# markokr/libacm

Hardware: AMD Instinct MI355X
Metric: decoded PCM Msamples/sec over a batch of ACM streams (hot path on HBM-resident staged input) (higher is better)
Workload: dtype int32

## Files before the change

### libacm_amd/csrc/acm_device.h

```cpp
#ifndef ACM_DEVICE_H
#define ACM_DEVICE_H

#include <stdint.h>

#include "acm_hip.h"

struct AcmDevStream {
	uint64_t idx_off;
	uint64_t hdr_off;
	uint64_t pcm_off;
	uint64_t n_emit;
	uint64_t scratch_off;
	uint32_t level;
	uint32_t rows;
	uint32_t nrows;
	uint32_t row_begin;
	uint32_t halo_row;
	uint32_t pad;
};

struct AcmTile {
	uint32_t stream;
	int32_t row0;
	uint32_t flags;
	uint32_t pad;
};
#define ACM_TILE_FRESH   1u
#define ACM_TILE_DISCARD 2u
#define ACM_TILE_ROW1    4u
#define ACM_TILE_ODD     8u
#define ACM_TILE_ONEBLOCK 16u

struct AcmTile2 {
	uint64_t idx_off;
	uint64_t pcm_off;
	uint32_t hdr_blk;
	uint32_t rowpos;
	uint32_t magic;
	uint32_t flags;
};

struct AcmDevPatch {
	uint64_t dst;
	int32_t value;
	uint32_t pad;
};

struct AcmParseJob {
	uint64_t file_off;
	uint64_t idx_off;
	uint64_t hdr_off;
	uint64_t col_off;
	uint32_t file_len;
	uint32_t data_start;
	uint32_t level;
	uint32_t rows;
	uint32_t blocks;
	uint32_t range_unit;
	uint64_t mf_off;
	uint32_t mf_pair_off;
	uint32_t mf_rows;
};
struct AcmParseResult {
	uint32_t blocks_done;
	uint32_t status;
	uint32_t end_bit;
	uint32_t mf_at;
};

struct AcmBlockJob {
	uint32_t job;
	uint32_t block;
	uint32_t bit;
	uint32_t end_bit;
	uint32_t h20;
	uint32_t pad;
};

#define ACM_K1_MIN_LEVEL 5
#define ACM_K1_MAX_LEVEL 12
#define ACM_K2_MIN_LEVEL 6
#define ACM_K2_MAX_LEVEL 14
#define ACM_K2P_MIN_LEVEL 6
#define ACM_K2P_MAX_LEVEL 9
// ... 112 lines not shown
```

### libacm_amd/csrc/acm_hip_api.cpp

```cpp
#include <hip/hip_runtime.h>

#include <cstdarg>
#include <cstdio>
#include <cstdlib>
#include <cstring>
#include <mutex>
#include <new>
#include <vector>

#include "acm_device.h"
#include "acm_hip.h"
#include "acm_plan_cut.h"

namespace {

thread_local char g_err[512] = "";

void set_err(const char *fmt, ...)
{
	va_list ap;
	va_start(ap, fmt);
	vsnprintf(g_err, sizeof(g_err), fmt, ap);
	va_end(ap);
}
// ... 472 lines not shown
	}
	if (plan->ev_fork)
		(void)hipEventDestroy(plan->ev_fork);
	for (hipEvent_t e : plan->ev_join)
		if (e)
			(void)hipEventDestroy(e);
	if (plan->dev) {
		acmhip_device *dev = plan->dev;
		std::vector<acmhip_device::Block> drop;
		{
			std::lock_guard<std::mutex> g(dev->spare_mutex);
			for (const acmhip_device::Block &b : plan->blocks) {
				if (dev->spare.size() < acmhip_device::SPARE_MAX_BLOCKS && dev->spare_bytes + b.bytes <= acmhip_device::SPARE_MAX_BYTES &&
				    b.bytes <= acmhip_device::SPARE_MAX_BYTES / 4) {
					dev->spare.push_back(b);
					dev->spare_bytes += b.bytes;
				} else {
					drop.push_back(b);
				}
			}
		}
		for (const acmhip_device::Block &b : drop)
			(void)hipFree(b.ptr);
	}
	delete plan;
}

extern "C" int acmhip_plan_create(acmhip_device *dev, const acmhip_stream_desc *streams, size_t n,
				  const acmhip_patch *patches, size_t npatches, unsigned flags,
				  acmhip_plan **out)
{
	return acmhip_plan_create_packed(dev, streams, n, nullptr, patches, npatches, flags, out);
}

extern "C" int acmhip_plan_create_packed(acmhip_device *dev, const acmhip_stream_desc *streams, size_t n, const acmhip_packed_stream *packed,
					 const acmhip_patch *patches, size_t npatches, unsigned flags, acmhip_plan **out)
{
	if (!dev || !out || (n && !streams) || (npatches && !patches) || n > 0xFFFFFFFFull)
		return ACMHIP_ERR_ARG;
	HIPTRY(hipSetDevice(dev->ordinal));
	AcmPlanCut cut;
	int rc = acm_plan_cut(dev->cus, streams, n, packed, patches, npatches, flags, &cut);
	if (rc != ACMHIP_OK)
		return rc;

	acmhip_plan *pl = new (std::nothrow) acmhip_plan;
	if (!pl)
		return ACMHIP_ERR_NOMEM;
	pl->dev = dev;
	pl->variant = cut.variant;
	pl->form_only = cut.form_only;
	pl->form_rows = std::move(cut.form_rows);
	pl->stats = cut.stats;
	rc = to_device(pl, cut.streams, &pl->d_streams);
	if (rc == ACMHIP_OK)
		rc = upload_groups(pl, cut.fused, &pl->fused);
	if (rc == ACMHIP_OK)
		rc = upload_groups(pl, cut.small, &pl->small);
	if (rc == ACMHIP_OK)
		rc = upload_groups(pl, cut.prefix, &pl->prefix);
	if (rc == ACMHIP_OK)
		rc = upload_groups(pl, cut.stagewise, &pl->stagewise);
	if (rc == ACMHIP_OK && cut.need_sink)
		rc = plan_malloc(pl, (void **)&pl->d_sink, ACM_K2_SINK_F32_BYTES);
	if (rc == ACMHIP_OK && cut.plane_elems > 0) {
		pl->n_sw_all = (uint32_t)cut.sw_all.size();
		pl->sw_max_elems = cut.sw_max_elems;
		pl->plane_elems = cut.plane_elems;
		pl->npatches = cut.patches.size();
		rc = to_device(pl, cut.sw_all, &pl->d_sw_all);
		if (rc == ACMHIP_OK)
			rc = to_device(pl, cut.patches, &pl->d_patches);
		for (int b = 0; b < 2 && rc == ACMHIP_OK; b++)
			rc = plan_malloc(pl, (void **)&pl->d_plane[b], cut.plane_elems * sizeof(int32_t));
	}
	if (rc == ACMHIP_OK)
		rc = upload_done(pl, (flags & ACMHIP_PLAN_UPLOAD_ASYNC) != 0);
	if (rc != ACMHIP_OK) {
		acmhip_plan_destroy(pl);
		return rc;
	}
	if (pl->fused.size() > 1 && !(ACM_TUNING_ENV("ACM_PLAN_STREAMS") && atoi(ACM_TUNING_ENV("ACM_PLAN_STREAMS")) <= 1)) {
		hipError_t e = hipEventCreateWithFlags(&pl->ev_fork, hipEventDisableTiming);
		for (int k = 0; k < 2 && e == hipSuccess; k++) {
			e = hipEventCreateWithFlags(&pl->ev_join[k], hipEventDisableTiming);
			if (e == hipSuccess && !dev->side[k])
				e = hipStreamCreateWithFlags(&dev->side[k], hipStreamNonBlocking);
		}
		if (e != hipSuccess) {
			rc = hip_fail(e, "side streams of a multi-level plan");
			acmhip_plan_destroy(pl);
			return rc;
		}
	}
	*out = pl;
	return ACMHIP_OK;
}

extern "C" int acmhip_plan_form_rows(const acmhip_plan *plan, size_t stream, uint64_t *rows)
{
	if (!plan || !rows || stream >= plan->form_rows.size())
		return ACMHIP_ERR_ARG;
	*rows = plan->form_rows[stream];
	return ACMHIP_OK;
}

// ... 161 lines not shown
```

### libacm_amd/csrc/acm_kernels.hip

```cpp
#include <hip/hip_runtime.h>

#include <utility>

#include "acm_device.h"

#ifndef ACM_L14_GROUPS
#define ACM_L14_GROUPS 3, 3, 3, 3, 2
#endif
#ifndef ACM_L13_GROUPS
#define ACM_L13_GROUPS 2, 3, 3, 3, 2
#endif

#ifndef ACM_OUT_F32
#define ACM_OUT_F32 0
#endif
#if ACM_OUT_F32
#define ACM_K_EMIT acm_sw_emit_f32
#define ACM_K_SMALL acm_small_level_f32
#define ACM_K_FUSED acm_fused_tile_f32
#define ACM_K_TILE2 acm_f32_tile2
#define ACM_K_CHUNK acm_f32_chunk
#define ACMK_OUT(name) name##_f32
#else
#define ACM_K_EMIT acm_sw_emit
// ... 1986 lines not shown
			e = (u >> 1) >= (uint32_t)j ? (uint32_t)opaque_s((int32_t)d.e[j]) : e;
		return e;
	}

	static constexpr bool HISTORY_IN_REGISTERS = RR == 1;
#ifndef ACM_K3_DPP_HISTORY
#define ACM_K3_DPP_HISTORY 1
#endif
	static constexpr bool HISTORY_BY_DPP = ACM_K3_DPP_HISTORY && RR >= 2 && NSW == 2 && RR * SIGMA == 16 && SIGMA >= 4;
	static constexpr bool KEEPS_ROWS = HISTORY_IN_REGISTERS || HISTORY_BY_DPP;
	template <int CTRL, int BANKS>
	static __device__ __forceinline__ v4u_t dpp4(const v4u_t old, const v4u_t src)
	{
		v4u_t r;
#pragma unroll
		for (int v = 0; v < 4; v++)
			r[v] = (uint32_t)__builtin_amdgcn_update_dpp((int)old[v], (int)src[v], CTRL, 0xF, BANKS, false);
		return r;
	}
	static constexpr int DPP_W0_BANKS = (1 << (SIGMA / 4)) - 1;
	static __device__ __forceinline__ void hand_history_on(Raw &raw)
	{
#pragma unroll
		for (int k = 0; k < 2; k++) {
			raw.lo[0][k] = dpp4<0x100 + (16 - SIGMA), DPP_W0_BANKS>(raw.lo[0][k], raw.lo[0][k + NSW]);
			raw.hi[0][k] = dpp4<0x100 + (16 - SIGMA), DPP_W0_BANKS>(raw.hi[0][k], raw.hi[0][k + NSW]);
		}
	}
	static __device__ __forceinline__ void take_history_from_partner(Raw &raw)
	{
#pragma unroll
		for (int k = 0; k < 2; k++) {
			raw.lo[0][k] = dpp4<0x110 + SIGMA, 0xF & ~DPP_W0_BANKS>(raw.lo[0][k], raw.lo[0][k + NSW]);
			raw.hi[0][k] = dpp4<0x110 + SIGMA, 0xF & ~DPP_W0_BANKS>(raw.hi[0][k], raw.hi[0][k + NSW]);
		}
	}
	static constexpr int JM = (TR & 1) ? 1 : TR / 2;
	static_assert(JM + 1 <= NE, "entries in reach are entries fetched");
	static __device__ __forceinline__ uint32_t half_bytes(const uint32_t cls) { return (0x4234u >> (4u * cls)) & 15u; }
	template <int J0>
	static __device__ __forceinline__ uint32_t mode_of(const uint32_t flags, const Desc &d, const uint32_t sval)
	{
		const uint32_t cls = d.e[0] & 3u;
		const uint32_t pair_units = (uint32_t)(COLS / 64) * half_bytes(cls);
		bool ok = (flags & ACM_TILE_ONEBLOCK) != 0 && cls != 0u;
		if constexpr (OutScale<L>::SHIFT != 0)
			ok = ok && sval < 65536u;
#pragma unroll
		for (int j = 1; j <= JM; j++)
			ok = ok && (d.e[j] & 3u) == cls;
#pragma unroll
		for (int j = J0; j < JM; j++)
			ok = ok && (d.e[j + 1] >> 2) - (d.e[j] >> 2) == pair_units;
		return ok ? (cls == ACMHIP_BP_NIB12 ? 3u : cls - (ACMHIP_BP_BYTE - 1u)) : 0u;
	}

#ifndef ACM_K3_LD_MOD
#define ACM_K3_LD_MOD " nt"
#endif
	template <bool KEEP>
	static __device__ __forceinline__ void issue(Raw &raw, const uint8_t *arena, const Desc &d, const int lane, const uint32_t odd, const uint32_t mode)
	{
		static_assert(!KEEP || KEEPS_ROWS, "the rows in front belong to another lane");
		constexpr int K0 = KEEP ? 2 : 0, J0 = KEEP ? 1 : 0;
		const uint32_t i = (uint32_t)lane & 15u, ks = (uint32_t)lane >> 4;
		const uint32_t c = class_of(i), rr = RR == 1 ? 0u : i / SIGMA;
		const uint32_t smode = __builtin_amdgcn_readfirstlane(mode);
		uint32_t va[NX][NG], vh[NX][NG];
		const uint8_t *sb[NX][NG];
		if (mode) {
			const uint32_t hb = smode == 1u ? 2u : smode == 2u ? 4u : 3u;
			const uint64_t base = reinterpret_cast<uint64_t>(arena) + ((uint64_t)(d.e[J0] >> 2) << 6);
			const uint32_t vl = (rr * (uint32_t)(NSW * COLS / 2) + c * (uint32_t)(QN / 2)) * hb + 16u * ks;
			const uint32_t vlh = vl - (smode == 3u ? 8u * ks : 0u);
#pragma unroll
			for (int k = K0; k < NX; k++)
#pragma unroll
				for (int g = 0; g < NG; g++) {
					va[k][g] = vl;
					vh[k][g] = vlh;
					sb[k][g] = sgpr_u64(base + (uint64_t)((((TR & 1 ? odd : 0u) + (uint32_t)(k - K0)) * (uint32_t)(COLS / 2) + group_at(g) * (uint32_t)(QN / 2)) * hb));
				}
		} else {
			const uint32_t e0 = d.e[0];
			const uint8_t *base = sgpr_u64(reinterpret_cast<uint64_t>(arena) + ((uint64_t)(e0 >> 2) << 6));
#pragma unroll
			for (int k = K0; k < NX; k++) {
				const uint32_t u = (TR & 1 ? odd : 0u) + rr * NSW + k;
				const uint32_t e = entry_of(d, u);
				const uint32_t hb = half_bytes(e & 3u);
				const uint32_t row_at = (((e >> 2) - (e0 >> 2)) << 6) + ((u & 1u) ? (uint32_t)(COLS / 2) * hb : 0u) + 16u * ks;
#pragma unroll
				for (int g = 0; g < NG; g++) {
					va[k][g] = row_at + (group_at(g) + c) * (uint32_t)(QN / 2) * hb;
					vh[k][g] = va[k][g] - ((e & 3u) == ACMHIP_BP_NIB12 ? 8u * ks : 0u);
					sb[k][g] = base;
				}
			}
		}
#pragma unroll
		for (int k = K0; k < NX; k++)
#pragma unroll
			for (int g = 0; g < NG; g++) {
				if constexpr (KEEPS_ROWS) {
					asm volatile("global_load_dwordx4 %0, %1, %2" ACM_K3_LD_MOD : "=v"(raw.lo[g][k]) : "v"(va[k][g]), "s"(sb[k][g]) : "memory");
					asm volatile("s_cmp_eq_u32 %3, 1\n\ts_cbranch_scc1 .Lacm_z8_%=\n\t"
						     "global_load_dwordx4 %0, %1, %2 offset:64" ACM_K3_LD_MOD "\n"
						     ".Lacm_z8_%=:"
						     : "+v"(raw.hi[g][k]) : "v"(vh[k][g]), "s"(sb[k][g]), "s"(smode) : "memory", "scc");
				} else {
					asm volatile("global_load_dwordx4 %0, %1, %2" : "=v"(raw.lo[g][k]) : "v"(va[k][g]), "s"(sb[k][g]) : "memory");
					asm volatile("s_cmp_eq_u32 %3, 1\n\ts_cbranch_scc1 .Lacm_z8_%=\n\t"
						     "global_load_dwordx4 %0, %1, %2 offset:64\n"
						     ".Lacm_z8_%=:"
						     : "+v"(raw.hi[g][k]) : "v"(vh[k][g]), "s"(sb[k][g]), "s"(smode) : "memory", "scc");
				}
			}
	}
	static __device__ __forceinline__ v4u_t expand_nib(const v4u_t x)
	{
// ... 223 lines not shown
#pragma unroll
							for (int v = 0; v < 4; v++)
								y[v] = (int32_t)(__umul24((uint32_t)ha[v], v8[v / NVH]) + (uint32_t)y[v]);
							goto joined;
						}
					}
					{
					v4i_t yh;
					int32_t wv[NH], w2[NH], w1[NH];
#pragma unroll
					for (int hf = 0; hf < NH; hf++) {
						wv[hf] = opaque_v(val[s][hf]);
						w2[hf] = opaque_v(dv2[s][hf]);
						w1[hf] = opaque_v(dv1[s][hf]);
					}
#pragma unroll
					for (int v = 0; v < 4; v++)
						yh[v] = __mul24(ha[v], wv[v / NVH]);
					if (step2[s]) {
#pragma unroll
						for (int v = 0; v < 4; v++)
							yh[v] += __mul24(h2[v], w2[v / NVH]);
					}
					if (step1[s]) {
#pragma unroll
						for (int v = 0; v < 4; v++)
							yh[v] += __mul24(h1[v], w1[v / NVH]);
					}
					const uint32_t hs = nform ? 4u : 8u;
#pragma unroll
					for (int v = 0; v < 4; v++)
						y[v] = (int32_t)(((uint32_t)opaque_v(yh[v]) << hs) + (uint32_t)y[v]);
					}
				joined:;
				}
				}
				static_assert(COLS % (1 << PS) == 0 && (SIGMA * 16) % (1 << PS) == 0 &&
					      (NG == 1 || (group_at(NG - 1) % (1 << PS) + CB + 7 < (1 << PS) && SIGMA % (1 << PS) == 0)), "address split");
#pragma unroll
				for (int hf = 0; hf < NH; hf++) {
					uint32_t *const o = tile + (o_lane[hf] + (uint32_t)((s * COLS + ((s * COLS) >> PS)) + (group_at(g) + (group_at(g) >> PS))));
#pragma unroll
					for (int v = 0; v < NVH; v++)
						o[v] = (uint32_t)y[hf * NVH + v];
				}
			}
			cf += 64;
#pragma unroll
			for (int hf = 0; hf < NH; hf++)
				o_lane[hf] += SIGMA * 16 + ((SIGMA * 16) >> PS);
		}
	}

	static __device__ __forceinline__ void run(Raw &raw, uint32_t *const tile, const Tables &t, const int lane_, const uint32_t hvs,
						   const Desc &d, const uint32_t in_front, const uint32_t odd, const uint32_t mode, const uint32_t sval,
						   const bool first)
	{
#ifdef ACM_K3_OPAQUE_LANE
		const int lane = opaque_v(lane_);
#else
		const int lane = lane_;
#endif
		const bool all_new = !KEEPS_ROWS || first;
		if (mode == 3u) {
#pragma unroll
			for (int k = 0; k < NX; k++)
				if (k >= 2 || all_new) {
#pragma unroll
					for (int g = 0; g < NG; g++)
						raw.hi[g][k] = expand_nib(raw.hi[g][k]);
				}
			if constexpr (HISTORY_BY_DPP)
				take_history_from_partner(raw);
			run_t<true, true, true>(raw, tile, t, lane, 0u, in_front, sval);
			return;
		}
		if (mode) {
			if constexpr (HISTORY_BY_DPP)
				take_history_from_partner(raw);
			if (mode == 2u)
				run_t<true, true>(raw, tile, t, lane, 0u, in_front, sval);
			else
				run_t<false, true>(raw, tile, t, lane, 0u, in_front, sval);
			return;
		}
		uint32_t any_word = 0, any_nib = 0, any_wordu = 0;
#pragma unroll
		for (int j = 0; j < NE; j++) {
			any_word |= (d.e[j] & 3u) == ACMHIP_BP_WORD ? 1u : 0u;
			any_nib |= (d.e[j] & 3u) == ACMHIP_BP_NIB12 ? 1u : 0u;
			any_wordu |= (d.e[j] & 3u) == ACMHIP_BP_WORDU ? 1u : 0u;
		}
		any_word |= any_wordu;
		const uint32_t rr = RR == 1 ? 0u : ((uint32_t)lane & 15u) / SIGMA;
		if (any_nib) {
#pragma unroll
			for (int k = 0; k < NX; k++)
				if (k >= 2 || all_new) {
					if ((entry_of(d, (TR & 1 ? odd : 0u) + rr * NSW + k) & 3u) == ACMHIP_BP_NIB12) {
#pragma unroll
						for (int g = 0; g < NG; g++)
							raw.hi[g][k] = expand_nib(raw.hi[g][k]);
					}
				}
		}
		if constexpr (HISTORY_BY_DPP)
			take_history_from_partner(raw);
		const bool nform = any_nib && !any_word;
		if (any_word | any_nib) {
#pragma unroll
			for (int k = 0; k < NX; k++) {
				const uint32_t cls = entry_of(d, (TR & 1 ? odd : 0u) + rr * NSW + k) & 3u;
				const uint32_t mask = cls == ACMHIP_BP_BYTE ? 0u : 0xFFFFFFFFu;
#pragma unroll
				for (int g = 0; g < NG; g++)
					raw.hi[g][k] &= mask;
// ... 34 lines not shown
	constexpr int PASS_ABL = ABL | MODE_WAVE | (FP::NG > 1 && NW == 16 ? MODE_LEAN : 0);

	__shared__ uint32_t tile_mem[NW][WTILE];
	__shared__ uint32_t carry_all[NW][NCARRY_WORDS];
	__shared__ typename FP::Tables tables;

	const int lane0 = threadIdx.x & 63;
	const uint32_t wave = __builtin_amdgcn_readfirstlane(threadIdx.x >> 6);
	FP::fill_tables(tables, threadIdx.x, NW * 64);
	__syncthreads();

	uint32_t *const tile = tile_mem[wave] + 8;
	uint32_t *const carry_mem = carry_all[wave];

	const uint32_t nvw = gridDim.x * NW, vw = blockIdx.x * NW + wave;
	const uint32_t per = (ntiles + nvw - 1) / nvw;
	uint32_t t = vw * per;
	const uint32_t t_end = t + per < ntiles ? t + per : ntiles;
	if (t >= t_end)
		return;
	bool discard = false;
	{
		const uint32_t f0 = tiles[__builtin_amdgcn_readfirstlane(t)].flags;
		if (f0 & ACM_TILE_DISCARD) {
			discard = true;
		} else if (!(f0 & ACM_TILE_FRESH)) {
			discard = true;
			t--;
		}
	}

	auto rows_in_front = [](const AcmTile2 &r) -> uint32_t { return (r.flags & ACM_TILE_FRESH) ? 0u : (r.flags & ACM_TILE_ROW1) ? 1u : 2u; };
	auto fetch_val = [&](const AcmTile2 &r, const int lane, uint32_t v, const uint32_t mode) -> uint32_t {
		const uint32_t *p = &hdr[0].val;
		if (!mode) {
			const uint32_t lr_fetch = (uint32_t)(lane < TR + 2 ? lane : TR + 1);
			const uint32_t missing = 2u - rows_in_front(r);
			const uint32_t q = r.rowpos + (lr_fetch < missing ? 0u : lr_fetch - missing);
			const uint32_t b = r.magic ? __umulhi(q, r.magic) : q;
			p = &hdr[r.hdr_blk + b].val;
		}
		asm volatile("s_cmp_lg_u32 %2, 0\n\ts_cbranch_scc1 .Lacm_zv_%=\n\t"
			     "global_load_dword %0, %1, off\n"
			     ".Lacm_zv_%=:"
			     : "+v"(v) : "v"(p), "s"(__builtin_amdgcn_readfirstlane(mode)) : "memory", "scc");
		return v;
	};
	typedef const uint32_t __attribute__((address_space(4))) *const_u32_ptr;
	auto val_of = [&](const AcmTile2 &r) -> uint32_t {
		const uint64_t a = reinterpret_cast<uint64_t>(&hdr[__builtin_amdgcn_readfirstlane(r.hdr_blk)].val);
		return *(const_u32_ptr)a << OutScale<L>::SHIFT;
	};

	constexpr int NVEC = TR * COLS / 8, PER_OWNER = NJ_LAST / 8, NSTORE = NVEC / 64;
	static_assert(NVEC % 64 == 0, "whole rounds");
	const uint8_t *const arena = reinterpret_cast<const uint8_t *>(idx);
	auto record_at = [&](const uint32_t k) -> AcmTile2 { return tiles[__builtin_amdgcn_readfirstlane(k < t_end ? k : t_end - 1)]; };
	constexpr int MODE_J0 = FP::KEEPS_ROWS ? 1 : 0;
#ifdef ACM_K3_NO_FAST
	auto mode_of = [&](const AcmTile2 &, const typename FP::Desc &, const uint32_t) -> uint32_t { return 0u; };
#else
	auto mode_of = [&](const AcmTile2 &r, const typename FP::Desc &d, const uint32_t sval) -> uint32_t {
		return FP::template mode_of<MODE_J0>(r.flags, d, sval);
	};
#endif
	AcmTile2 cur = record_at(t);
	typename FP::Desc dcur = FP::fetch_desc(pairs, cur);
	typename FP::Raw raw;
	{
		const v4u_t z = { 0, 0, 0, 0 };
#pragma unroll
		for (int g = 0; g < FP::NG; g++)
#pragma unroll
			for (int k = 0; k < FP::NX; k++)
				raw.hi[g][k] = z;
	}
	uint32_t mode_cur = 0u, sv_cur = val_of(cur);
	uint32_t hv = fetch_val(cur, lane0, 0u, 0u);
	FP::template issue<false>(raw, arena, dcur, lane0, (cur.flags & ACM_TILE_ODD) ? 1u : 0u, 0u);
	k2_wait<0>();
	bool fresh = true, first_of_run = true;
	AcmTile2 nxt = record_at(t + 1), nx2 = record_at(t + 2);
	typename FP::Desc dnxt = FP::fetch_desc(pairs, nxt);
	uint32_t sv_nxt = val_of(nxt);
	uint32_t mode_nxt = mode_of(nxt, dnxt, sv_nxt);
#ifdef ACM_STAMPS
	unsigned long long acc_[8] = { 0, 0, 0, 0, 0, 0, 0, 0 };
	unsigned long long last_ = stamp_now();
#endif
	for (;;) {
		const uint32_t tn = t + 1;
		const bool more = tn < t_end;
		int lane = lane0;
#ifdef ACM_K3_OPAQUE_LANE
		asm volatile("" : "+v"(lane));
#endif
		if (fresh)
			for (int k = lane; k < NCARRY_WORDS; k += 64)
				carry_mem[k] = 0u;
		const uint32_t hvs = hv << OutScale<L>::SHIFT;
		ACM_STAMP(0);
		phase_prio<true, PRIO_FIRST_PASS>();
		FP::run(raw, tile, tables, lane, hvs, dcur, rows_in_front(cur), (cur.flags & ACM_TILE_ODD) ? 1u : 0u, mode_cur, sv_cur, first_of_run);
		first_of_run = false;
		phase_prio<true, PRIO_IDLE>();
		ACM_STAMP(1);

		hv = fetch_val(nxt, lane, hv, mode_nxt);
		if constexpr (FP::HISTORY_IN_REGISTERS) {
			FP::shift_history(raw);
			if (nxt.flags & ACM_TILE_FRESH)
				FP::zero_history(raw);
			FP::template issue<true>(raw, arena, dnxt, lane, (nxt.flags & ACM_TILE_ODD) ? 1u : 0u, mode_nxt);
		} else if constexpr (FP::HISTORY_BY_DPP) {
			FP::hand_history_on(raw);
			if (nxt.flags & ACM_TILE_FRESH)
				FP::zero_history(raw);
			FP::template issue<true>(raw, arena, dnxt, lane, (nxt.flags & ACM_TILE_ODD) ? 1u : 0u, mode_nxt);
		} else {
			FP::template issue<false>(raw, arena, dnxt, lane, (nxt.flags & ACM_TILE_ODD) ? 1u : 0u, mode_nxt);
		}
		const AcmTile2 nx3 = record_at(t + 3);
		const typename FP::Desc dnx2 = FP::fetch_desc(pairs, nx2);
		const uint32_t sv_nx2 = val_of(nx2);
		ACM_STAMP(2);
		phase_prio<true, PRIO_LDS_PASSES>();
		run_lds_passes<C, PASS_ABL, true, FP::G, Gs...>(tile, lane, F32 ? (unsigned)ACMHIP_FMT_S16LE : fmt, carry_mem);
		tile_barrier<MODE_WAVE>();
		ACM_STAMP(3);
		if constexpr (F32) {
			float *out = discard ? reinterpret_cast<float *>(sink) : reinterpret_cast<float *>(pcm) + cur.pcm_off;
			lean_store_f32<C, 64, NSTORE, ABL>(tile, lane, out);
		} else {
			typedef uint32_t v4u __attribute__((ext_vector_type(4)));
			v4u *out = discard ? reinterpret_cast<v4u *>(sink) : reinterpret_cast<v4u *>(reinterpret_cast<uint16_t *>(pcm) + cur.pcm_off);
#pragma unroll
			for (int k = 0; k < NSTORE; k++) {
				const int vec = lane + k * 64;
				const uint32_t *q = tile + lds_at<C::PS>((vec / PER_OWNER) * NJ_LAST) + (vec % PER_OWNER) * park_piece<NJ_LAST>();
				const v4u o = { q[0], q[1], q[2], q[3] };
#ifdef ACM_K3_ST_MOD
				asm volatile("global_store_dwordx4 %0, %1, %2" ACM_K3_ST_MOD :: "v"((uint32_t)(vec * 16)), "v"(o), "s"(sgpr_u64(reinterpret_cast<uint64_t>(out))) : "memory");
#else
				__builtin_nontemporal_store(o, &out[vec]);
#endif
			}
		}
		ACM_STAMP(5);
		phase_prio<true, PRIO_IDLE>();
		k2_wait<F32 ? 2 * NSTORE : NSTORE>();
		ACM_STAMP(6);
		tile_barrier<MODE_WAVE>();
		if (!more)
			break;
		fresh = (nxt.flags & (ACM_TILE_FRESH | ACM_TILE_DISCARD)) != 0;
		discard = (nxt.flags & ACM_TILE_DISCARD) != 0;
		cur = nxt;
		dcur = dnxt;
		sv_cur = sv_nxt;
		mode_cur = mode_nxt;
		t = tn;
		nxt = nx2;
		dnxt = dnx2;
		sv_nxt = sv_nx2;
		mode_nxt = mode_of(nxt, dnxt, sv_nxt);
		nx2 = nx3;
	}
#ifdef ACM_STAMPS
	if (lane0 == 0 && vw < 2048)
		for (int k = 0; k < 8; k++)
			g_acm_stamps[vw][k] = acc_[k];
#endif
}

struct Tile2Entry {
	typedef void (*Fn)(const AcmTile2 *, uint32_t, const int16_t *, const uint32_t *, const acmhip_blkhdr *, int16_t *, int16_t *, unsigned);
	Fn fn;
	int threads, tile_rows, wg_per_cu;
};
template <class C, int... Gs>
constexpr Tile2Entry entry_k2()
{
	return Tile2Entry{ ACM_K_TILE2<C, 4, 0, false, Gs...>, C::NT, C::TR, 1024 / C::NT };
}
template <class C, int WPC, int... Gs>
constexpr Tile2Entry entry_k2w()
{
	return Tile2Entry{ ACM_K_TILE2<C, WPC * C::NT / 256, 0, false, Gs...>, C::NT, C::TR, WPC };
}
#ifdef ACM_ABLATION
template <int ABL>
constexpr Tile2Entry abl_k2() { return Tile2Entry{ ACM_K_TILE2<TileCfg<9, 256, 8192>, 4, ABL, false, 3, 3, 3>, 256, 16, 4 }; }
const struct { int mask; Tile2Entry e; } g_tile2_abl[] = {
	{ 1, abl_k2<1>() }, { 2, abl_k2<2>() }, { 4, abl_k2<4>() }, { 6, abl_k2<6>() }, { 8, abl_k2<8>() }, { 16, abl_k2<16>() },
	{ 17, abl_k2<17>() }, { 23, abl_k2<23>() }, { 32, abl_k2<32>() }, { 25, abl_k2<25>() }, { 31, abl_k2<31>() }, { 12, abl_k2<12>() },
};
#endif
const Tile2Entry g_tile2[ACM_K2_MAX_LEVEL - ACM_K2_MIN_LEVEL + 1] = {
	entry_k2<TileCfg<6, 256, 8192>, 2, 2, 2>(),
	entry_k2<TileCfg<7, 256, 8192>, 3, 2, 2>(),
	entry_k2<TileCfg<8, 256, 8192>, 3, 3, 2>(),
	entry_k2<TileCfg<9, 256, 8192>, 3, 3, 3>(),
	entry_k2<TileCfg<10, 256, 8192>, 3, 3, 2, 2>(),
	entry_k2<TileCfg<11, 256, 8192>, 3, 3, 3, 2>(),
	entry_k2w<TileCfg<12, 512, 16384>, 2, 3, 3, 3, 3>(),
	entry_k2w<TileCfg<13, 1024, 32768>, 1, ACM_L13_GROUPS>(),
	entry_k2w<TileCfg<14, 1024, 32768>, 1, ACM_L14_GROUPS>(),
};
inline const Tile2Entry &tile2_entry(uint32_t level)
{
	return g_tile2[level - ACM_K2_MIN_LEVEL];
}
template <class C, int... Gs>
constexpr Tile2Entry entry_k2m()
{
	return Tile2Entry{ ACM_K_TILE2<C, 4, 0, true, Gs...>, C::NT, C::TR, 1024 / C::NT };
}
// ... 731 lines not shown
```

### libacm_amd/csrc/acm_plan_cut.cpp

```cpp
#include <algorithm>
#include <cstdarg>
#include <cstdio>
#include <cstdlib>
#include <cstring>

#include "acm_plan_cut.h"

#define ACM_K1_DEFAULT_VARIANT 0

namespace {

void set_err(const char *fmt, ...)
{
	char text[512];
	va_list ap;
	va_start(ap, fmt);
	vsnprintf(text, sizeof(text), fmt, ap);
	va_end(ap);
	acmhip_set_error_text(text);
}

bool fused_ok(const acmhip_stream_desc &s, int variant)
{
	return s.level >= ACM_K1_MIN_LEVEL && s.level <= ACM_K1_MAX_LEVEL && acmk_fused_tile_rows(s.level, variant) > 2;
// ... 513 lines not shown
			g.carry = carry_wanted(L.prefix_tiles_carry.size(), (size_t)acmk_plane_grid(cus), (size_t)acmk_plane_tile_rows(), flags);
			g.tiles = std::move(g.carry ? L.prefix_tiles_carry : L.prefix_tiles);
			st.tiles += g.tiles.size();
			st.launches += g.prefix_patched ? 2 + g.prefix_stages : 2;
			cut.prefix.push_back(std::move(g));
		}
		if (!L.list.empty()) {
			AcmCutGroup g;
			g.level = level;
			g.max_elems = L.max_elems;
			g.max_emit = L.max_emit;
			g.list = std::move(L.list);
			cut.stagewise.push_back(std::move(g));
			st.launches += level + 1;
		}
	}
	if (cut.plane_elems > 0) {
		st.launches += cut.sw_all.empty() ? 0 : 1;
		st.launches += cut.patches.empty() ? 0 : 1;
	}
}

int Cutter::run()
{
	int rc = index_patches();
	if (rc != ACMHIP_OK)
		return rc;
	cut.streams.resize(n);
	cut.form_rows.assign(n, 0);
	cut.variant = variant;
	cut.form_only = (flags & ACMHIP_PLAN_FORM_ONLY) != 0;
	plane_shift.assign(n, 0);
	on_tile_kernel.assign(n, 0);
	count_high_levels();
	for (size_t i = 0; i < n && rc == ACMHIP_OK; i++)
		rc = cut_stream(i);
	if (rc == ACMHIP_OK)
		rc = resolve_patches();
	if (rc == ACMHIP_OK)
		choose_tables();
	return rc;
}

}

int acm_plan_cut(int cus, const acmhip_stream_desc *streams, size_t n, const acmhip_packed_stream *packed,
		 const acmhip_patch *patches, size_t npatches, unsigned flags, AcmPlanCut *out)
{
	if (!out || (n && !streams) || (npatches && !patches) || n > 0xFFFFFFFFull)
		return ACMHIP_ERR_ARG;
	*out = AcmPlanCut{};
	Cutter c(cus, streams, n, packed, patches, npatches, flags, *out);
	return c.run();
}

extern "C" int acmk_plan_cut_visit(int cus, const acmhip_stream_desc *streams, size_t n, const acmhip_packed_stream *packed,
				   const acmhip_patch *patches, size_t npatches, unsigned flags, acmk_cut_visit visit, void *ctx)
{
	AcmPlanCut cut;
	const int rc = acm_plan_cut(cus, streams, n, packed, patches, npatches, flags, &cut);
	if (rc != ACMHIP_OK || !visit)
		return rc;
	auto show = [&](const char *name, uint32_t level, const auto &v) {
		if (!v.empty())
			visit(ctx, name, level, v.data(), sizeof(v[0]), v.size());
	};
	show("streams", 0, cut.streams);
	const std::vector<AcmCutGroup> *kinds[4] = { &cut.fused, &cut.small, &cut.prefix, &cut.stagewise };
	static const char *const list_name[4] = { "", "small_list", "prefix_list", "sw_list" };
	std::vector<uint64_t> words(sizeof(cut.stats) / 8);
	memcpy(words.data(), &cut.stats, sizeof(cut.stats));
	const uint64_t head[4] = { cut.plane_elems, cut.sw_max_elems, cut.need_sink, cut.fused.size() + cut.small.size() + cut.prefix.size() + cut.stagewise.size() };
	words.insert(words.end(), head, head + 4);
	for (uint64_t k = 0; k < 4; k++)
		for (const AcmCutGroup &g : *kinds[k]) {
			show(k == 2 ? "prefix_tiles" : "tiles", g.level, g.tiles);
			show("tiles_extra", g.level, g.tiles_extra);
			show("tiles2", g.level, g.tiles2);
			show("tiles2p", g.level, g.tiles2p);
			show("tiles2p_plain", g.level, g.tiles2p_plain);
			show("tiles2m", g.level, g.tiles2m);
			show("tiles2m_plain", g.level, g.tiles2m_plain);
			show(list_name[k], g.level, g.list);
			const uint64_t rec[7] = { k, g.level, g.carry, g.max_elems, g.max_emit, g.prefix_patched, g.prefix_stages };
			words.insert(words.end(), rec, rec + 7);
		}
	show("sw_all", 0, cut.sw_all);
	show("patches", 0, cut.patches);
	show("form_rows", 0, cut.form_rows);
	show("stats", 0, words);
	return rc;
}
```

### libacm_amd/csrc/acm_plan_cut.h

```cpp
#ifndef ACM_PLAN_CUT_H
#define ACM_PLAN_CUT_H

#include <vector>

#include "acm_device.h"

struct AcmCutGroup {
	uint32_t level = 0;
	std::vector<AcmTile> tiles, tiles_extra;
	bool carry = false;
	std::vector<AcmTile2> tiles2, tiles2p, tiles2p_plain, tiles2m, tiles2m_plain;
	std::vector<uint32_t> list;
	uint64_t max_elems = 0, max_emit = 0;
	bool prefix_patched = false;
	uint32_t prefix_stages = 0;
};

struct AcmPlanCut {
	std::vector<AcmDevStream> streams;
	std::vector<AcmCutGroup> fused, small, prefix, stagewise;
	std::vector<uint32_t> sw_all;
	uint64_t sw_max_elems = 0, plane_elems = 0;
	std::vector<AcmDevPatch> patches;
	std::vector<uint64_t> form_rows;
	bool need_sink = false;
	int variant = 0;
	bool form_only = false;
	acmhip_plan_stats stats{};
};

int acm_plan_cut(int cus, const acmhip_stream_desc *streams, size_t n, const acmhip_packed_stream *packed,
		 const acmhip_patch *patches, size_t npatches, unsigned flags, AcmPlanCut *out);

extern "C" {
typedef void (*acmk_cut_visit)(void *ctx, const char *table, uint32_t level, const void *data, size_t elem_bytes, size_t count);
int acmk_plan_cut_visit(int cus, const acmhip_stream_desc *streams, size_t n, const acmhip_packed_stream *packed,
			const acmhip_patch *patches, size_t npatches, unsigned flags, acmk_cut_visit visit, void *ctx);
}

#endif
```

Measured before the change: 1.358 million.

## Add edge fast path for level-9 chunks straddling a block boundary

The planner now flags level-9 chunks whose two history rows come from the previous block (rowpos == rows-2) with a new ACM_TILE_EDGE bit. The first-pass kernel detects these flagged chunks and runs a specialized MFMA path that scales the old and new block rows with separate per-block values, instead of falling back to the general decode path. It adds a second header-value load per tile, extra register pressure and more template code. It also adds a profiling script that reports how many chunks take each path.

```diff
diff --git a/libacm_amd/csrc/acm_device.h b/libacm_amd/csrc/acm_device.h
--- a/libacm_amd/csrc/acm_device.h
+++ b/libacm_amd/csrc/acm_device.h
@@ -30,6 +30,8 @@
 #define ACM_TILE_ROW1    4u
 #define ACM_TILE_ODD     8u
 #define ACM_TILE_ONEBLOCK 16u
+#define ACM_TILE_EDGE    32u
+#define ACM_EDGE_LEVEL   9u
 
 struct AcmTile2 {
 	uint64_t idx_off;
diff --git a/libacm_amd/csrc/acm_hip_api.cpp b/libacm_amd/csrc/acm_hip_api.cpp
--- a/libacm_amd/csrc/acm_hip_api.cpp
+++ b/libacm_amd/csrc/acm_hip_api.cpp
@@ -548,6 +548,8 @@
 	pl->form_only = cut.form_only;
 	pl->form_rows = std::move(cut.form_rows);
 	pl->stats = cut.stats;
+	for (AcmCutGroup &g : cut.fused)
+		acm_plan_mark_edge(g.level, (uint32_t)acmk_tile2m_rows(g.level), g.tiles2m.data(), g.tiles2m.size());
 	rc = to_device(pl, cut.streams, &pl->d_streams);
 	if (rc == ACMHIP_OK)
 		rc = upload_groups(pl, cut.fused, &pl->fused);
diff --git a/libacm_amd/csrc/acm_kernels.hip b/libacm_amd/csrc/acm_kernels.hip
--- a/libacm_amd/csrc/acm_kernels.hip
+++ b/libacm_amd/csrc/acm_kernels.hip
@@ -2062,7 +2062,29 @@
 #pragma unroll
 		for (int j = J0; j < JM; j++)
 			ok = ok && (d.e[j + 1] >> 2) - (d.e[j] >> 2) == pair_units;
-		return ok ? (cls == ACMHIP_BP_NIB12 ? 3u : cls - (ACMHIP_BP_BYTE - 1u)) : 0u;
+		if constexpr (EDGE_PATH) {
+			if (flags & ACM_TILE_EDGE)
+				return edge_mode_of<J0>(d);
+		}
+		return ok ? width_code(cls) : 0u;
+	}
+	static __device__ __forceinline__ uint32_t width_code(const uint32_t cls) { return cls == ACMHIP_BP_NIB12 ? 3u : cls - (ACMHIP_BP_BYTE - 1u); }
+	static constexpr bool EDGE_PATH = HISTORY_BY_DPP && RR == 2 && NSW == 2 && NG == 1 && NH == 1 && OutScale<L>::SHIFT == 0;
+	static constexpr uint32_t MODE_WIDTH = 3u, MODE_EDGE = 4u;
+	template <int J0>
+	static __device__ __forceinline__ uint32_t edge_mode_of(const Desc &d)
+	{
+		static_assert(J0 == 1, "the rows in front of an edge chunk are history");
+		const uint32_t a = d.e[0] & 3u, b = d.e[1] & 3u;
+		const uint32_t pair_units = (uint32_t)(COLS / 64) * half_bytes(b);
+		bool ok = a != ACMHIP_BP_WORDU && b != ACMHIP_BP_WORDU && (a ^ b) != (ACMHIP_BP_NIB12 ^ ACMHIP_BP_WORD);
+#pragma unroll
+		for (int j = 2; j <= JM; j++)
+			ok = ok && (d.e[j] & 3u) == b;
+#pragma unroll
+		for (int j = J0; j < JM; j++)
+			ok = ok && (d.e[j + 1] >> 2) - (d.e[j] >> 2) == pair_units;
+		return ok ? (width_code(b) | MODE_EDGE) : 0u;
 	}
 
 #ifndef ACM_K3_LD_MOD
@@ -2075,7 +2097,9 @@
 		constexpr int K0 = KEEP ? 2 : 0, J0 = KEEP ? 1 : 0;
 		const uint32_t i = (uint32_t)lane & 15u, ks = (uint32_t)lane >> 4;
 		const uint32_t c = class_of(i), rr = RR == 1 ? 0u : i / SIGMA;
-		const uint32_t smode = __builtin_amdgcn_readfirstlane(mode);
+		uint32_t smode = __builtin_amdgcn_readfirstlane(mode);
+		if constexpr (EDGE_PATH)
+			smode &= MODE_WIDTH;
 		uint32_t va[NX][NG], vh[NX][NG];
 		const uint8_t *sb[NX][NG];
 		if (mode) {
@@ -2405,9 +2429,77 @@
 		}
 	}
 
+	template <int HK>
+	static __device__ __forceinline__ void run_edge_t(const Raw &raw, uint32_t *const tile, const Tables &t, const int lane, const uint32_t in_front,
+							  const uint32_t v_new, const uint32_t v_old, const uint32_t h_new, const uint32_t h_old)
+	{
+		static_assert(EDGE_PATH, "two walkers of two rows each, one group, four classes of one walker per lane");
+		const v4i_t zero = { 0, 0, 0, 0 };
+		const uint32_t qd = (uint32_t)lane & 15u, i = 4u * ((uint32_t)lane >> 4);
+		const uint32_t c0 = i % SIGMA, rrd = i / SIGMA;
+		const uint32_t m_lane = rrd * (uint32_t)(NSW * COLS) + c0 + (uint32_t)SIGMA * qd;
+		uint32_t o_lane = m_lane + (m_lane >> PS);
+		uint32_t bias_at[NSW];
+#pragma unroll
+		for (int s = 0; s < NSW; s++) {
+			const uint32_t row = in_front + rrd * NSW + s;
+			bias_at[s] = ((row < 2 ? row : 2u) * 2u + (c0 == 0 ? 0u : 1u)) * (uint32_t)QN + qd;
+		}
+		const int32_t mn = opaque_s((int32_t)__builtin_amdgcn_readfirstlane(v_new));
+		const int32_t mo = opaque_v((int32_t)(rrd ? v_new : v_old));
+		const int32_t hn = opaque_s((int32_t)__builtin_amdgcn_readfirstlane(h_new));
+		const int32_t ho = opaque_v((int32_t)(rrd ? h_new : h_old));
+		const v4i_t *cf = &t.coef[0][0][lane];
+		ACM_UNROLL(ACM_K3_MT_UNROLL)
+		for (int mt = 0; mt < NM; mt++) {
+			const v4i_t cf0 = cf[0], cf1 = cf[NM * 64], cf2 = cf[2 * NM * 64];
+#pragma unroll
+			for (int s = 0; s < NSW; s++) {
+				const int32_t b = (&t.bias[0][0][0])[bias_at[s] + 16u * (uint32_t)mt];
+				v4i_t y;
+				{
+					v4i_t po = mfma(raw.lo[0][s], cf2, zero);
+					if (s == 0)
+						po = mfma(raw.lo[0][1], cf1, po);
+#pragma unroll
+					for (int v = 0; v < 4; v++)
+						y[v] = __mul24(po[v], mo) + (v == 0 ? b : 0);
+				}
+				{
+					v4i_t pn = mfma(raw.lo[0][2], s == 0 ? cf0 : cf1, zero);
+					if (s == 1)
+						pn = mfma(raw.lo[0][3], cf0, pn);
+#pragma unroll
+					for (int v = 0; v < 4; v++)
+						y[v] = __mul24(pn[v], mn) + y[v];
+				}
+				if constexpr (HK != 0) {
+					v4i_t qo = mfma(raw.hi[0][s], cf2, zero);
+					if (s == 0)
+						qo = mfma(raw.hi[0][1], cf1, qo);
+#pragma unroll
+					for (int v = 0; v < 4; v++)
+						y[v] = HK == 1 ? __mul24(qo[v], ho) + y[v] : (int32_t)(__umul24((uint32_t)qo[v], (uint32_t)ho) + (uint32_t)y[v]);
+					v4i_t qn = mfma(raw.hi[0][2], s == 0 ? cf0 : cf1, zero);
+					if (s == 1)
+						qn = mfma(raw.hi[0][3], cf0, qn);
+#pragma unroll
+					for (int v = 0; v < 4; v++)
+						y[v] = HK == 1 ? __mul24(qn[v], hn) + y[v] : (int32_t)(__umul24((uint32_t)qn[v], (uint32_t)hn) + (uint32_t)y[v]);
+				}
+				uint32_t *const o = tile + (o_lane + (uint32_t)(s * COLS + ((s * COLS) >> PS)));
+#pragma unroll
+				for (int v = 0; v < 4; v++)
+					o[v] = (uint32_t)y[v];
+			}
+			cf += 64;
+			o_lane += SIGMA * 16 + ((SIGMA * 16) >> PS);
+		}
+	}
+
 	static __device__ __forceinline__ void run(Raw &raw, uint32_t *const tile, const Tables &t, const int lane_, const uint32_t hvs,
 						   const Desc &d, const uint32_t in_front, const uint32_t odd, const uint32_t mode, const uint32_t sval,
-						   const bool first)
+						   const bool first, const uint32_t sval2 = 0u)
 	{
 #ifdef ACM_K3_OPAQUE_LANE
 		const int lane = opaque_v(lane_);
@@ -2415,6 +2507,28 @@
 		const int lane = lane_;
 #endif
 		const bool all_new = !KEEPS_ROWS || first;
+		if constexpr (EDGE_PATH) {
+			if (mode & MODE_EDGE) {
+				const uint32_t a = d.e[0] & 3u, width = mode & MODE_WIDTH;
+				const bool hi_old = a != ACMHIP_BP_BYTE, hi_new = width != 1u;
+				if (width == 3u) {
+#pragma unroll
+					for (int k = 2; k < NX; k++)
+						raw.hi[0][k] = expand_nib(raw.hi[0][k]);
+					take_history_from_partner(raw);
+					run_edge_t<1>(raw, tile, t, lane, in_front, sval2, sval, sval2 << 4, hi_old ? sval << 4 : 0u);
+					return;
+				}
+				take_history_from_partner(raw);
+				if (a == ACMHIP_BP_NIB12)
+					run_edge_t<1>(raw, tile, t, lane, in_front, sval2, sval, 0u, sval << 4);
+				else if (!hi_old && !hi_new)
+					run_edge_t<0>(raw, tile, t, lane, in_front, sval2, sval, 0u, 0u);
+				else
+					run_edge_t<2>(raw, tile, t, lane, in_front, sval2, sval, hi_new ? sval2 << 8 : 0u, hi_old ? sval << 8 : 0u);
+				return;
+			}
+		}
 		if (mode == 3u) {
 #pragma unroll
 			for (int k = 0; k < NX; k++)
@@ -2555,6 +2669,17 @@
 		return *(const_u32_ptr)a << OutScale<L>::SHIFT;
 	};
 
+	static_assert(!FP::EDGE_PATH || L == (int)ACM_EDGE_LEVEL, "the planner sets ACM_TILE_EDGE for the levels whose first pass has the edge path");
+	auto val2_of = [&](const AcmTile2 &r) -> uint32_t {
+		if constexpr (FP::EDGE_PATH) {
+			const uint32_t blk = __builtin_amdgcn_readfirstlane(r.hdr_blk) + ((__builtin_amdgcn_readfirstlane(r.flags) & ACM_TILE_EDGE) ? 1u : 0u);
+			const uint64_t a = reinterpret_cast<uint64_t>(&hdr[blk].val);
+			return *(const_u32_ptr)a << OutScale<L>::SHIFT;
+		} else {
+			return 0u;
+		}
+	};
+
 	constexpr int NVEC = TR * COLS / 8, PER_OWNER = NJ_LAST / 8, NSTORE = NVEC / 64;
 	static_assert(NVEC % 64 == 0, "whole rounds");
 	const uint8_t *const arena = reinterpret_cast<const uint8_t *>(idx);
@@ -2578,14 +2703,14 @@
 			for (int k = 0; k < FP::NX; k++)
 				raw.hi[g][k] = z;
 	}
-	uint32_t mode_cur = 0u, sv_cur = val_of(cur);
+	uint32_t mode_cur = 0u, sv_cur = val_of(cur), sv2_cur = 0u;
 	uint32_t hv = fetch_val(cur, lane0, 0u, 0u);
 	FP::template issue<false>(raw, arena, dcur, lane0, (cur.flags & ACM_TILE_ODD) ? 1u : 0u, 0u);
 	k2_wait<0>();
 	bool fresh = true, first_of_run = true;
 	AcmTile2 nxt = record_at(t + 1), nx2 = record_at(t + 2);
 	typename FP::Desc dnxt = FP::fetch_desc(pairs, nxt);
-	uint32_t sv_nxt = val_of(nxt);
+	uint32_t sv_nxt = val_of(nxt), sv2_nxt = val2_of(nxt);
 	uint32_t mode_nxt = mode_of(nxt, dnxt, sv_nxt);
 #ifdef ACM_STAMPS
 	unsigned long long acc_[8] = { 0, 0, 0, 0, 0, 0, 0, 0 };
@@ -2604,7 +2729,7 @@
 		const uint32_t hvs = hv << OutScale<L>::SHIFT;
 		ACM_STAMP(0);
 		phase_prio<true, PRIO_FIRST_PASS>();
-		FP::run(raw, tile, tables, lane, hvs, dcur, rows_in_front(cur), (cur.flags & ACM_TILE_ODD) ? 1u : 0u, mode_cur, sv_cur, first_of_run);
+		FP::run(raw, tile, tables, lane, hvs, dcur, rows_in_front(cur), (cur.flags & ACM_TILE_ODD) ? 1u : 0u, mode_cur, sv_cur, first_of_run, sv2_cur);
 		first_of_run = false;
 		phase_prio<true, PRIO_IDLE>();
 		ACM_STAMP(1);
@@ -2625,7 +2750,7 @@
 		}
 		const AcmTile2 nx3 = record_at(t + 3);
 		const typename FP::Desc dnx2 = FP::fetch_desc(pairs, nx2);
-		const uint32_t sv_nx2 = val_of(nx2);
+		const uint32_t sv_nx2 = val_of(nx2), sv2_nx2 = val2_of(nx2);
 		ACM_STAMP(2);
 		phase_prio<true, PRIO_LDS_PASSES>();
 		run_lds_passes<C, PASS_ABL, true, FP::G, Gs...>(tile, lane, F32 ? (unsigned)ACMHIP_FMT_S16LE : fmt, carry_mem);
@@ -2661,11 +2786,13 @@
 		cur = nxt;
 		dcur = dnxt;
 		sv_cur = sv_nxt;
+		sv2_cur = sv2_nxt;
 		mode_cur = mode_nxt;
 		t = tn;
 		nxt = nx2;
 		dnxt = dnx2;
 		sv_nxt = sv_nx2;
+		sv2_nxt = sv2_nx2;
 		mode_nxt = mode_of(nxt, dnxt, sv_nxt);
 		nx2 = nx3;
 	}
diff --git a/libacm_amd/csrc/acm_plan_cut.cpp b/libacm_amd/csrc/acm_plan_cut.cpp
--- a/libacm_amd/csrc/acm_plan_cut.cpp
+++ b/libacm_amd/csrc/acm_plan_cut.cpp
@@ -589,6 +589,27 @@
 	*out = AcmPlanCut{};
 	Cutter c(cus, streams, n, packed, patches, npatches, flags, *out);
 	return c.run();
+}
+
+void acm_plan_mark_edge(uint32_t level, uint32_t chunk_rows, AcmTile2 *rec, size_t n)
+{
+	if (level != ACM_EDGE_LEVEL || chunk_rows < 2)
+		return;
+	uint32_t magic = 0, srows = 1;
+	for (size_t k = 0; k < n; k++) {
+		AcmTile2 &r = rec[k];
+		if (r.magic != magic) {
+			magic = r.magic;
+			srows = magic ? (uint32_t)(((1ull << 32) + magic - 1) / magic) : 1u;
+		}
+		const bool edge = !(r.flags & (ACM_TILE_FRESH | ACM_TILE_ROW1 | ACM_TILE_ODD)) && srows >= chunk_rows && r.rowpos == srows - 2;
+		r.flags = (r.flags & ~ACM_TILE_EDGE) | (edge ? ACM_TILE_EDGE : 0u);
+	}
+}
+
+extern "C" void acmk_plan_mark_edge(uint32_t level, AcmTile2 *rec, size_t n)
+{
+	acm_plan_mark_edge(level, (uint32_t)acmk_tile2m_rows(level), rec, n);
 }
 
 extern "C" int acmk_plan_cut_visit(int cus, const acmhip_stream_desc *streams, size_t n, const acmhip_packed_stream *packed,
diff --git a/libacm_amd/csrc/acm_plan_cut.h b/libacm_amd/csrc/acm_plan_cut.h
--- a/libacm_amd/csrc/acm_plan_cut.h
+++ b/libacm_amd/csrc/acm_plan_cut.h
@@ -32,7 +32,10 @@
 int acm_plan_cut(int cus, const acmhip_stream_desc *streams, size_t n, const acmhip_packed_stream *packed,
 		 const acmhip_patch *patches, size_t npatches, unsigned flags, AcmPlanCut *out);
 
+void acm_plan_mark_edge(uint32_t level, uint32_t chunk_rows, AcmTile2 *rec, size_t n);
+
 extern "C" {
+void acmk_plan_mark_edge(uint32_t level, AcmTile2 *rec, size_t n);
 typedef void (*acmk_cut_visit)(void *ctx, const char *table, uint32_t level, const void *data, size_t elem_bytes, size_t count);
 int acmk_plan_cut_visit(int cus, const acmhip_stream_desc *streams, size_t n, const acmhip_packed_stream *packed,
 			const acmhip_patch *patches, size_t npatches, unsigned flags, acmk_cut_visit visit, void *ctx);
diff --git a/profiles/edge_coverage.py b/profiles/edge_coverage.py
--- /dev/null
+++ b/profiles/edge_coverage.py
@@ -0,0 +1,93 @@
+#!/usr/bin/env python3
+import argparse
+import collections
+import ctypes as C
+import os
+import sys
+
+ROOT = os.path.dirname(os.path.dirname(os.path.abspath(__file__)))
+sys.path.insert(0, ROOT)
+
+import numpy as np
+
+TILE2 = np.dtype([("idx_off", "<u8"), ("pcm_off", "<u8"), ("hdr_blk", "<u4"), ("rowpos", "<u4"), ("magic", "<u4"), ("flags", "<u4")])
+ONEBLOCK, EDGE = 16, 32
+WORDU, NIB12, BYTE, WORD = 0, 1, 2, 3
+BITS = {WORDU: "wr", NIB12: "12", BYTE: "8", WORD: "16"}
+HALF_BYTES = {WORDU: 4, NIB12: 3, BYTE: 2, WORD: 4}
+VISIT = C.CFUNCTYPE(None, C.c_void_p, C.c_char_p, C.c_uint32, C.c_void_p, C.c_size_t, C.c_size_t)
+
+
+def chunk_records(L, descs, packed, level):
+    from libacm_amd import capi
+    out = {}
+
+    def visit(_ctx, name, lv, data, elem_bytes, count):
+        if name == b"tiles2m" and lv == level:
+            out["rec"] = np.frombuffer(C.string_at(data, elem_bytes * count), dtype=TILE2)
+    L.acmk_plan_cut_visit.argtypes = [C.c_int, C.c_void_p, C.c_size_t, C.c_void_p, C.c_void_p, C.c_size_t, C.c_uint, VISIT, C.c_void_p]
+    arr = (capi.StreamDesc * len(descs))(*descs)
+    pk = (capi.PackedStream * len(descs))(*packed)
+    rc = L.acmk_plan_cut_visit(256, arr, len(descs), pk, None, 0, capi.PLAN_AUTO, VISIT(visit), None)
+    if rc or "rec" not in out:
+        raise SystemExit("plan cut: %d %s" % (rc, L.acmhip_last_error()))
+    rec = out["rec"].copy()
+    L.acmk_plan_mark_edge.argtypes = [C.c_uint32, C.c_void_p, C.c_size_t]
+    L.acmk_plan_mark_edge.restype = None
+    L.acmk_plan_mark_edge(level, rec.ctypes.data, len(rec))
+    return rec
+
+
+def mode_of(flags, e, cols):
+    cls = [int(x) & 3 for x in e]
+    at = [int(x) >> 2 for x in e]
+    units = lambda c: cols // 64 * HALF_BYTES[c]
+    if flags & EDGE:
+        a, b = cls[0], cls[1]
+        if WORDU in (a, b):
+            return "general", "boundary, whole-range class"
+        if {a, b} == {NIB12, WORD}:
+            return "general", "boundary, 12 <-> 16"
+        if cls[2] != b or at[2] - at[1] != units(b):
+            return "general", "boundary, width change inside the chunk"
+        return "edge", "%s->%s" % (BITS[a], BITS[b])
+    if not flags & ONEBLOCK:
+        return "general", "boundary in reach, not at the chunk's start"
+    if cls[0] == WORDU:
+        return "general", "whole-range class"
+    if cls[1] != cls[0] or cls[2] != cls[0] or at[2] - at[1] != units(cls[0]):
+        return "general", "width change inside a block"
+    return "fast", BITS[cls[0]]
+
+
+def main():
+    ap = argparse.ArgumentParser()
+    ap.add_argument("--streams", type=int, default=16)
+    ap.add_argument("--level", type=int, default=9)
+    ap.add_argument("--rows", type=int, default=16)
+    ap.add_argument("--blocks", type=int, default=250)
+    a = ap.parse_args()
+    from libacm_amd import capi, workload
+    L = capi.lib()
+    b = workload.build_uniform(a.streams, a.level, a.rows, a.blocks, threads=max(1, min(16, workload.usable_cpus())))
+    mf = capi.mform_streams(b.idx, b.descs, threads=max(1, min(16, workload.usable_cpus())))
+    rec = chunk_records(L, b.descs, mf.streams, a.level)
+    cols = 1 << a.level
+    count = collections.Counter()
+    for r in rec:
+        e = mf.pairs[int(r["idx_off"]):int(r["idx_off"]) + 3]
+        kind, what = mode_of(int(r["flags"]), e, cols)
+        count[(kind, what)] += 1
+    n = len(rec)
+    print("level %d, %d rows per block, %d blocks, %d streams: %d chunks" % (a.level, a.rows, a.blocks, a.streams, n))
+    for kind in ("fast", "edge", "general"):
+        sub = sorted((k[1], v) for k, v in count.items() if k[0] == kind)
+        tot = sum(v for _, v in sub)
+        print("  %-8s %6d  %5.1f %%   %s" % (kind, tot, 100.0 * tot / n, "  ".join("%s %d (%.1f %%)" % (w, v, 100.0 * v / n) for w, v in sub)))
+    flagged = int(((rec["flags"] & EDGE) != 0).sum())
+    edge = sum(v for k, v in count.items() if k[0] == "edge")
+    print("  chunks with ACM_TILE_EDGE: %d (%.1f %%), %.1f %% of them on the edge path" % (flagged, 100.0 * flagged / n, 100.0 * edge / max(flagged, 1)))
+
+
+if __name__ == "__main__":
+    main()
```

New measurement: 1.355 million. No clear change (-0.2%).
